# TFMV/quiver

Measured on AMD Instinct MI355X. Metric: flat_cosine_qps_recall_1.0, higher is better.
Workload: dtype f64; 1 GPU; flat cosine scan 10000000x768 fp32, k=10, single query per step, recall 1.0 (exact, bit-identical to the CPU oracle); rows_total=10000000, rows_per_gpu=10000000, dim=768, k=10, scan_streams=1, device=AMD Radeon Graphics (gfx950:sramecc+:xnack-), cus=256, rccl_ranks_seen=0

## Files before the change

### include/qv.h

```cpp
#ifndef QV_H
#define QV_H

#include <stdint.h>
#include <stddef.h>

#ifdef __cplusplus
extern "C" {
#endif

#define QV_ABI_VERSION 4

typedef struct qv_index qv_index;

typedef enum qv_metric {
    QV_COSINE      = 0,
    QV_L2          = 1,
    QV_L2SQ        = 2,
    QV_DOT         = 3,
    QV_L1          = 4,
    QV_COSINE_F32  = 5,
    QV_L2_F32      = 6,
    QV_DOT_F32     = 7,
    QV_L2SQ_F64    = 8,
    QV_METRIC_COUNT = 9
// ... 154 lines not shown
                                       uint32_t candidate_tiles);
int qv_scan_bound8_applies_mq(int metric, uint32_t dim, uint32_t rows, uint32_t nq, uint32_t k, int mode, int plane_mode_mq, int has_plane8);
int qv_scan_bound8_applies_filtered(int metric, uint32_t dim, uint32_t rows, uint32_t nq, uint32_t k, int mode, int plane_mode_filtered, int has_plane8,
                                    uint32_t candidate_tiles);
int qv_scan_bound8_applies(int metric, uint32_t dim, uint32_t rows, uint32_t nq, uint32_t k, int mode, int plane_mode, int has_plane8);
int qv_scan_bound_interval8(int metric, uint32_t dim, int64_t isum, double sq, double qn, double qres, double rn, float rscale8, float rres8, float* d_lo, float* d_hi);
int qv_scan_quantize_row8(uint32_t dim, const float* row, int8_t* out_bytes, float* out_scale, float* out_res);
int qv_scan_bound_applies(int metric, uint32_t dim, uint32_t rows, uint32_t nq, uint32_t k, int mode, int has_plane);
int qv_scan_bound_applies_filtered(int metric, uint32_t dim, uint32_t rows, uint32_t nq, uint32_t k, int mode, int has_plane, uint32_t candidate_tiles);
int qv_scan_route(int metric, uint32_t dim, uint32_t rows, uint32_t nq, uint32_t k, int cus, int tickets, int bound_mode, int plane_mode, int has_plane, int has_plane8,
                  uint32_t candidate_tiles);
int qv_scan_route_ex(int metric, uint32_t dim, uint32_t rows, uint32_t nq, uint32_t k, int cus, int tickets, int bound_mode, int plane_mode, int has_plane, int has_plane8,
                     uint32_t candidate_tiles, int plane_mode_filtered);
int qv_scan_bound_interval(int metric, uint32_t dim, float s, double qn, double rn, float rres, float* d_lo, float* d_hi);
int qv_scan_bound_interval_l2(uint32_t dim, float s, double qn, double rn, float rres, float* d_lo, float* d_hi);
#define QV_DEBUG_RNORM 0
#define QV_DEBUG_RRES  1
#define QV_DEBUG_PLANE 2
#define QV_DEBUG_ROWMAJ16 3
int qv_index_debug_read(qv_index* idx, int what, void* out, size_t bytes);

int qv_index_search_batched_device(qv_index* idx, const float* d_queries, uint32_t nq, uint32_t k,
                                   uint32_t* d_rows_out, float* d_dist_out, uint32_t* d_redo_flags_out, void* stream);

int qv_distance_rows(qv_index* idx, const float* query, const uint32_t* rows, uint32_t n, float* dist_out);
int qv_distance_rows_device(qv_index* idx, const float* d_query, const uint32_t* d_rows, uint32_t n,
                            float* d_dist_out, void* stream);

int qv_distance_pairs(qv_metric metric, const float* a, const float* b, uint32_t n, uint32_t dim,
                      float* dist_out, int device);
// ... 94 lines not shown
```

### quiver_amd/_lib.py

```python
from __future__ import annotations

import ctypes as C
import os

_HERE = os.path.dirname(os.path.abspath(__file__))
LIB_PATH = os.environ.get("QV_LIB_PATH") or os.path.join(_HERE, "lib", "libqv.so")

QV_OK = 0
QV_ERR_INVALID_ARG, QV_ERR_DIM_MISMATCH, QV_ERR_K_NOT_POSITIVE, QV_ERR_OUT_OF_RANGE = -1, -2, -3, -4
QV_ERR_NO_DEVICE, QV_ERR_DEVICE, QV_ERR_OOM, QV_ERR_UNSUPPORTED = -5, -6, -7, -8
QV_FLAG_ROWMAJOR = 1
QV_FLAG_BF16_ROWS = 2
QV_FLAG_NO_SCAN_PLANE = 4
QV_FLAG_L2_SCAN_PLANE = 8
QV_FLAG_GRAPH_PLANE = 16
QV_GRAPH_REJECT_AUTO, QV_GRAPH_REJECT_ALWAYS, QV_GRAPH_REJECT_NEVER = 0, 1, 2
QV_DEBUG_RNORM, QV_DEBUG_RRES, QV_DEBUG_PLANE, QV_DEBUG_ROWMAJ16 = 0, 1, 2, 3
QV_RULE_L2_PLANES = 0x101
QV_BOUND_SCAN_AUTO, QV_BOUND_SCAN_ALWAYS, QV_BOUND_SCAN_NEVER = 0, 1, 2
QV_FILTERED_BATCH_AUTO, QV_FILTERED_BATCH_ALWAYS, QV_FILTERED_BATCH_NEVER = 0, 1, 2
QV_COL_F64, QV_COL_U32 = 0, 1
QV_SET_AND, QV_SET_OR, QV_SET_ANDNOT = 0, 1, 2
QV_SHARDED_PEER_COPY = 1 << 32

# ... 65 lines not shown
    "qv_merge_topk_device": (C.c_int, [C.c_void_p, C.c_void_p, C.c_uint32, C.c_uint32, C.c_void_p, C.c_void_p, C.c_void_p]),
    "qv_merge_topk_shards_device": (C.c_int, [C.c_void_p, C.c_void_p, C.c_uint32, C.c_uint32, C.c_uint32, C.c_void_p, C.c_void_p, C.c_void_p]),
    "qv_index_set_filter": (C.c_int, [C.c_void_p, C.c_int]),
    "qv_index_set_filtered_batch": (C.c_int, [C.c_void_p, C.c_int, C.c_uint32]),
    "qv_index_filtered_batch_stats": (C.c_int, [C.c_void_p, C.POINTER(C.c_uint64)]),
    "qv_batched_applies_filtered": (C.c_int, [C.c_int, C.c_uint32, C.c_uint64, C.c_uint32, C.c_uint32, C.c_int, C.c_int, C.c_uint32]),
    "qv_batched_filter_route": (C.c_int, [C.c_int, C.c_uint32, C.c_uint64, C.c_uint32, C.c_uint32, C.c_int, C.c_int, C.c_int, _u32p, C.POINTER(C.c_int)]),
    "qv_batched_sample_plan": (C.c_int, [C.c_void_p, C.c_uint32, C.c_uint32, _u32p, _u32p, _u32p]),
    "qv_sharded_set_filter": (C.c_int, [C.c_void_p, C.c_int]),
    "qv_index_set_bound_scan": (C.c_int, [C.c_void_p, C.c_int]),
    "qv_sharded_set_bound_scan": (C.c_int, [C.c_void_p, C.c_int]),
    "qv_index_bound_scan_stats": (C.c_int, [C.c_void_p, C.POINTER(C.c_uint64)]),
    "qv_sharded_bound_scan_stats": (C.c_int, [C.c_void_p, C.POINTER(C.c_uint64)]),
    "qv_scan_bound_interval": (C.c_int, [C.c_int, C.c_uint32, C.c_float, C.c_double, C.c_double, C.c_float, _f32p, _f32p]),
    "qv_scan_bound_interval_l2": (C.c_int, [C.c_uint32, C.c_float, C.c_double, C.c_double, C.c_float, _f32p, _f32p]),
    "qv_index_set_bound_plane": (C.c_int, [C.c_void_p, C.c_int]),
    "qv_sharded_set_bound_plane": (C.c_int, [C.c_void_p, C.c_int]),
    "qv_index_bound_scan8_stats": (C.c_int, [C.c_void_p, C.POINTER(C.c_uint64)]),
    "qv_sharded_bound_scan8_stats": (C.c_int, [C.c_void_p, C.POINTER(C.c_uint64)]),
    "qv_index_set_bound_plane_filtered": (C.c_int, [C.c_void_p, C.c_int]),
    "qv_index_set_bound_plane_mq": (C.c_int, [C.c_void_p, C.c_int]),
    "qv_sharded_set_bound_plane_mq": (C.c_int, [C.c_void_p, C.c_int]),
    "qv_index_set_bound_plane_filtered_mq": (C.c_int, [C.c_void_p, C.c_int]),
    "qv_scan_bound8_applies_filtered_mq": (C.c_int, [C.c_int, C.c_uint32, C.c_uint32, C.c_uint32, C.c_uint32, C.c_int, C.c_int, C.c_int, C.c_uint32]),
    "qv_scan_bound8_applies_mq": (C.c_int, [C.c_int, C.c_uint32, C.c_uint32, C.c_uint32, C.c_uint32, C.c_int, C.c_int, C.c_int]),
    "qv_scan_bound8_applies_filtered": (C.c_int, [C.c_int, C.c_uint32, C.c_uint32, C.c_uint32, C.c_uint32, C.c_int, C.c_int, C.c_int, C.c_uint32]),
    "qv_scan_route_ex": (C.c_int, [C.c_int, C.c_uint32, C.c_uint32, C.c_uint32, C.c_uint32, C.c_int, C.c_int, C.c_int, C.c_int, C.c_int, C.c_int, C.c_uint32, C.c_int]),
    "qv_scan_bound8_applies": (C.c_int, [C.c_int, C.c_uint32, C.c_uint32, C.c_uint32, C.c_uint32, C.c_int, C.c_int, C.c_int]),
    "qv_scan_bound_interval8": (C.c_int, [C.c_int, C.c_uint32, C.c_int64, C.c_double, C.c_double, C.c_double, C.c_double, C.c_float, C.c_float, _f32p, _f32p]),
    "qv_scan_quantize_row8": (C.c_int, [C.c_uint32, C.c_void_p, C.c_void_p, _f32p, _f32p]),
# ... 88 lines not shown
```

### quiver_amd/csrc/qv_api.cpp

```cpp
#include "qv_api_internal.h"

#include <atomic>

namespace {
thread_local char g_err[512] = "";

}

int qv_fail(int code, const char* fmt, ...) {
    va_list ap; va_start(ap, fmt);
    vsnprintf(g_err, sizeof(g_err), fmt, ap);
    va_end(ap);
    return code;
}

namespace {

int acquire_ctx(qv_index* idx, SearchCtx** out) {
    {
        std::lock_guard<std::mutex> g(idx->ctx_mu);
        if (!idx->free_ctx.empty()) { *out = idx->free_ctx.back(); idx->free_ctx.pop_back(); return QV_OK; }
    }
    SearchCtx* c = new (std::nothrow) SearchCtx();
    if (!c) return fail(QV_ERR_OOM, "out of host memory");
// ... 1687 lines not shown
    return qv::host_quantize_row8(dim, row, out_bytes, out_scale, out_res);
}

int qv_scan_bound_interval(int metric, uint32_t dim, float s, double qn, double rn, float rres, float* d_lo, float* d_hi) {
    if (metric != QV_COSINE && metric != QV_DOT)
        return fail(QV_ERR_UNSUPPORTED, "the bound scan's metrics are cosine, dot and l2, and this function serves cosine and dot (l2: qv_scan_bound_interval_l2); got %d", metric);
    if (!d_lo || !d_hi || dim == 0) return fail(QV_ERR_INVALID_ARG, "d_lo/d_hi is null or dim is 0");
    return qv::host_bound_interval(metric, dim, s, qn, rn, rres, d_lo, d_hi);
}

int qv_scan_bound_interval_l2(uint32_t dim, float s, double qn, double rn, float rres, float* d_lo, float* d_hi) {
    if (!d_lo || !d_hi || dim == 0) return fail(QV_ERR_INVALID_ARG, "d_lo/d_hi is null or dim is 0");
    return qv::host_bound_interval(QV_L2, dim, s, qn, rn, rres, d_lo, d_hi);
}

int qv_index_debug_read(qv_index* idx, int what, void* out, size_t bytes) {
    if (!idx) return fail(QV_ERR_INVALID_ARG, "index is null");
    const int m = idx->metric;
    const bool f64norm = m == QV_COSINE || m == QV_DOT || m == QV_L2 || m == QV_L2SQ;
    const size_t tiles = ((size_t)idx->n_rows + 63) / 64;
    const void* src = nullptr; size_t need = 0;
    if (what == QV_DEBUG_RNORM) {
        if (!f64norm && m != QV_COSINE_F32) return fail(QV_ERR_UNSUPPORTED, "metric %d keeps no row norms", m);
        src = idx->d_rnorm; need = tiles * 64 * sizeof(double);
    } else if (what == QV_DEBUG_RRES) {
        if (!f64norm) return fail(QV_ERR_UNSUPPORTED, "metric %d keeps no bfloat16 residuals", m);
        src = idx->d_rres; need = tiles * 64 * sizeof(float);
    } else if (what == QV_DEBUG_PLANE) {
        if (!idx->wants_plane() || (tiles && !idx->d_bf16)) return fail(QV_ERR_UNSUPPORTED, "this index keeps no bfloat16 copy");
        src = idx->d_bf16; need = tiles * idx->bf16_tile_bytes();
// ... 183 lines not shown
```

### quiver_amd/csrc/qv_bound.h

```cpp
#pragma once
#include "qv_kernels.h"
#include "qv_filter.h"

namespace qv {

__host__ __device__ static inline double bound_scan_gamma(uint32_t dim) { return filter_gamma(dim, 0) * (1.0 + 1e-6) + 5e-7 + 1e-12; }

__host__ __device__ static inline bool bound_scan_norm_ok(double n, uint32_t dim) { return n >= (double)filter_tiny_norm(dim) && n < 1.0e18; }

constexpr double kBoundL2Theta = 1.2e-7, kBoundL2NormSlack = 2e-12;
__host__ __device__ __forceinline__ bool bound_l2_ends(double s, double m, double qn, double rn, float& d_lo, float& d_hi) {
    const double A = __builtin_fma(qn, qn, rn * rn);
    const double c = A - 2.0 * s, w = 2.0 * m + kBoundL2NormSlack * A;
    const double e_lo = c - w, e_hi = c + w;
    if (!(e_hi >= 0.0)) { d_lo = -__builtin_inff(); d_hi = __builtin_nanf(""); return false; }
    QConst qc; qc.qn = qn; qc.qn32 = 0.0f;
    d_lo = finalize<QV_L2>((e_lo > 0.0 ? e_lo : 0.0) * ((1.0 - kBoundL2Theta) * (1.0 - 1e-9)), qc, rn);
    d_hi = finalize<QV_L2>(e_hi * ((1.0 + kBoundL2Theta) * (1.0 + 1e-9)), qc, rn);
    return true;
}

template <int M>
__host__ __device__ __forceinline__ bool bound_scan_interval(float s, double qn, double rn, float rres, uint32_t dim, double gamma, float& d_lo, float& d_hi) {
    static_assert(M == QV_COSINE || M == QV_DOT || M == QV_L2, "the bound scan's metrics");
// ... 38 lines not shown
                                                              float& d_lo, float& d_hi) {
    static_assert(M == QV_COSINE || M == QV_DOT || M == QV_L2, "the bound scan's metrics");
    const double rr = (double)rres8, sc = (double)rscale;
    const bool sure = bound_scan_norm_ok(rn, dim) && bound_scan_norm_ok(qn, dim) && rr >= 0.0 && rr < 1.0e18 && qres >= 0.0 && qres < 1.0e18 &&
                      sq > 0.0 && sq < 1.0e36 && sc > 0.0 && sc < 1.0e36;
    if (!sure) { d_lo = -__builtin_inff(); d_hi = __builtin_nanf(""); return false; }
    const double s = sq * sc * (double)isum;
    const double m = (qn * rr + qres * (rn + rr) + 1e-12 * (qn + qres) * (rn + rr)) * (1.0 + 1e-9);
    if constexpr (M == QV_L2) return bound_l2_ends(s, m, qn, rn, d_lo, d_hi);
    QConst qc; qc.qn = qn; qc.qn32 = 0.0f;
    d_lo = finalize<M>(s + m, qc, rn);
    d_hi = finalize<M>(s - m, qc, rn);
    return true;
}

}
```

### quiver_amd/csrc/qv_bound_scan.hip

```cpp
#include "qv_kernels.h"
#include "qv_bound.h"

namespace qv {

typedef uint32_t u4 __attribute__((ext_vector_type(4)));
constexpr uint32_t kBoundCandCap = 4096;
constexpr uint32_t kBoundMaxDim = 4096;
struct BoundCtrl { uint32_t thr_inv, cand_cnt, ticket, flag; };

template <int U, bool QN>
__device__ __forceinline__ void bound_block(const u4* __restrict__ p, const float* __restrict__ q_lds, uint32_t s0, float& acc, double& qa) {
    u4 x[2 * U];
#pragma unroll
    for (int u = 0; u < U; u++) {
        x[2 * u] = __builtin_nontemporal_load(&p[(size_t)(s0 + u) * 128]);
        x[2 * u + 1] = __builtin_nontemporal_load(&p[(size_t)(s0 + u) * 128 + 32]);
    }
    __builtin_amdgcn_sched_barrier(0);
#pragma unroll
    for (int u = 0; u < U; u++) {
        const f4* qq = reinterpret_cast<const f4*>(q_lds + (size_t)(s0 + u) * 16);
#pragma unroll
        for (int h = 0; h < 2; h++) {
            const u4 w = x[2 * u + h];
// ... 123 lines not shown
        const uint32_t xs[4] = {x.x, x.y, x.z, x.w};
#pragma unroll
        for (int j = 0; j < 4; j++) {
            const bool c = xs[j] <= H && xs[j] != 0xFFFFFFFFu;
            const uint64_t m = __ballot(c);
            if (m) {
                uint32_t b0 = 0;
                if (lane == (uint32_t)__builtin_ctzll(m)) b0 = atomicAdd(cnt, (uint32_t)__builtin_popcountll(m));
                b0 = __builtin_amdgcn_readlane(b0, (uint32_t)__builtin_ctzll(m));
                const uint32_t slot = b0 + (uint32_t)__builtin_popcountll(m & ((1ull << lane) - 1ull));
                if (c && slot < kBoundCandCap) cand[slot] = i + (uint32_t)j;
            }
        }
    }
}
__global__ void __launch_bounds__(256)
k_bound_collect(const uint32_t* __restrict__ lo_all, uint32_t n , BoundCtrl* __restrict__ ctrl, uint32_t* __restrict__ cand,
                const uint32_t* __restrict__ gate = nullptr ) {
    if (gate != nullptr && *gate == 0u) return;
    const uint32_t inv = ctrl->thr_inv;
    if (inv == 0u) return;
    bound_collect(lo_all, n, ~inv, &ctrl->cand_cnt, cand);
}

template <int M, typename F>
__device__ __forceinline__ void bound_rescore_query(const IndexView& v, const float* __restrict__ query, uint32_t k, uint32_t cnt, bool has_H, const uint32_t* __restrict__ cand,
                                                    uint32_t* __restrict__ rows_out, float* __restrict__ dist_out, F decided) {
    using Q = typename MT<M>::Q;
    extern __shared__ __align__(16) unsigned char smem[];
    Q* q_lds = reinterpret_cast<Q*>(smem);
    uint64_t* wl = reinterpret_cast<uint64_t*>(smem + (((size_t)v.dim4 * 4 * sizeof(Q)) + 15) / 16 * 16);
    __shared__ double s_qn;
    const uint32_t lane = lane_id();
    const uint32_t wave = __builtin_amdgcn_readfirstlane(threadIdx.x >> 6);
    const uint32_t ns = cnt < kBoundCandCap ? cnt : kBoundCandCap, kth = k - 1;
    stage_query<M>(q_lds, query, v.dim, v.dim4);
    __syncthreads();
    const f4* tiles = reinterpret_cast<const f4*>(v.tiles);
// ... 24 lines not shown
        else list_insert(list, thr, key, kth, lane);
    }
    __syncthreads();
    wl[wave * 64 + lane] = list;
    __syncthreads();
    if (wave == 0) {
        for (uint32_t w = 1; w < kScanWaves; w++) list_insert(list, thr, lane < k ? wl[w * 64 + lane] : kDeadKey, kth, lane);
        if (lane < k) {
            const bool dead = list == kDeadKey;
            rows_out[lane] = dead ? 0xFFFFFFFFu : (uint32_t)list;
            dist_out[lane] = dead ? __uint_as_float(0x7F800000u) : unord_f32((uint32_t)(list >> 32));
        }
    }
}

constexpr uint32_t kBoundRescoreGrid = 64;
template <int M, bool P8 = false>
__global__ void __launch_bounds__(kScanBlock)
k_bound_rescore(IndexView v, const float* __restrict__ query, uint32_t k, BoundCtrl* __restrict__ ctrl, const uint32_t* __restrict__ cand,
                uint32_t* __restrict__ stats, uint32_t* __restrict__ rows_out, float* __restrict__ dist_out, uint32_t* gate, BoundCtrl* next,
                uint64_t* __restrict__ partial ) {
    if (gate != nullptr && *gate == 0u) return;
    using Q = typename MT<M>::Q;
    extern __shared__ __align__(16) unsigned char smem[];
    Q* q_lds = reinterpret_cast<Q*>(smem);
    const size_t q_bytes = (((size_t)v.dim4 * 4 * sizeof(Q)) + 15) / 16 * 16;
    uint64_t* wl = reinterpret_cast<uint64_t*>(smem + q_bytes);
    float* rbuf = reinterpret_cast<float*>(smem + q_bytes + (size_t)kScanWaves * 64 * sizeof(uint64_t));
    __shared__ double s_qn;
    __shared__ uint32_t s_last;
    const uint32_t cnt = ctrl->cand_cnt, thr_inv = ctrl->thr_inv;
    const uint32_t lane = lane_id();
    const uint32_t wave = __builtin_amdgcn_readfirstlane(threadIdx.x >> 6);
    const uint32_t ns = cnt < kBoundCandCap ? cnt : kBoundCandCap, kth = k - 1;
    const uint32_t active = std::max(1u, std::min((uint32_t)gridDim.x, (ns + kScanWaves - 1) / kScanWaves));
    const bool idle = blockIdx.x >= active;
    if (idle) {
        if (threadIdx.x == 0) s_last = atomicAdd(&ctrl->ticket, 1u) == gridDim.x - 1 ? 1u : 0u;
        __syncthreads();
        if (!s_last) return;
    }
    stage_query<M>(q_lds, query, v.dim, v.dim4);
    __syncthreads();
    if (wave == kScanWaves - 1) {
        double ma = 0.0;
        for (uint32_t i = 0; i < v.dim; i++) { const double a = (double)q_lds[i]; ma = __builtin_fma(a, a, ma); }
        if (lane == 0) s_qn = __builtin_sqrt(ma);
    }
    __syncthreads();
    const double qn = s_qn;
    const bool hand_back = cnt > kBoundCandCap || thr_inv == 0u || !bound_scan_norm_ok(qn, v.dim);
    uint64_t list = kDeadKey, thr = kDeadKey;
    if (!hand_back && !idle) {
        QConst qc; qc.qn = 0.0; qc.qn32 = 0.0f;
        if constexpr (M == QV_COSINE) qc.qn = qn;
        const f4* tiles = reinterpret_cast<const f4*>(v.tiles);
        f4* mine = reinterpret_cast<f4*>(rbuf + (size_t)wave * v.dim4 * 4);
        bool first = true;
        for (uint32_t i = blockIdx.x * kScanWaves + wave; i < ns; i += active * kScanWaves) {
            const uint32_t row = cand[i];
            const f4* src = tiles + (size_t)(row >> 6) * v.dim4 * 64 + (row & 63);
            double rn = 0.0;
            if constexpr (MT<M>::needs_rnorm) rn = v.rnorm[row];
            for (uint32_t c0 = 0; c0 < v.dim4; c0 += 256) {
                f4 x[4];
#pragma unroll
                for (uint32_t u = 0; u < 4; u++) { const uint32_t c = c0 + u * 64 + lane; if (c < v.dim4) x[u] = __builtin_nontemporal_load(&src[(size_t)c * 64]); }
#pragma unroll
                for (uint32_t u = 0; u < 4; u++) { const uint32_t c = c0 + u * 64 + lane; if (c < v.dim4) mine[c] = x[u]; }
            }
            __builtin_amdgcn_fence(__ATOMIC_RELEASE, "wavefront");
            __builtin_amdgcn_wave_barrier();
            __builtin_amdgcn_fence(__ATOMIC_ACQUIRE, "wavefront");
            typename MT<M>::A acc = 0;
            for (uint32_t c = 0; c < v.dim4; c++) {
                const f4 r = mine[c];
                const Q* qq = q_lds + (size_t)c * 4;
                acc1<M>(acc, qq[0], r.x); acc1<M>(acc, qq[1], r.y); acc1<M>(acc, qq[2], r.z); acc1<M>(acc, qq[3], r.w);
            }
            __builtin_amdgcn_fence(__ATOMIC_RELEASE, "wavefront");
            __builtin_amdgcn_wave_barrier();
            const uint64_t key = lane == 0 ? make_key(finalize<M>(acc, qc, rn), row) : kDeadKey;
            if (first) { list = wave_sort64(key, lane); thr = readlane64(list, kth); first = false; }
            else list_insert(list, thr, key, kth, lane);
        }
    }
    wl[wave * 64 + lane] = list;
    __syncthreads();
    if (wave == 0 && !idle) {
        if (!hand_back) {
            for (uint32_t w = 1; w < kScanWaves; w++) list_insert(list, thr, lane < k ? wl[w * 64 + lane] : kDeadKey, kth, lane);
            uint64_t* out = partial + (size_t)blockIdx.x * k;
            if (lane < k) (void)atomicExch(reinterpret_cast<unsigned long long*>(&out[lane]), (unsigned long long)list);
            asm volatile("s_waitcnt vmcnt(0)" ::: "memory");
        }
        uint32_t last = 0;
        if (lane == 0) last = atomicAdd(&ctrl->ticket, 1u) == gridDim.x - 1 ? 1u : 0u;
        last = __builtin_amdgcn_readfirstlane(last);
        if (lane == 0) s_last = last;
    }
    __syncthreads();
    if (!s_last) return;
    if (threadIdx.x == 0) {
        ctrl->ticket = 0;
        if constexpr (P8) {
            stats[kBound8StatsWord] = cnt;
            if (hand_back) (void)atomicAdd(&stats[kBound8StatsWord + 1], 1u);
            (void)atomicAdd(&stats[kBound8StatsWord + 2], 1u);
            if (!hand_back) { stats[0] = cnt; (void)atomicAdd(&stats[2], 1u); next->flag = 0u; }
        } else {
            stats[0] = cnt;
            if (hand_back) (void)atomicAdd(&stats[1], 1u);
            (void)atomicAdd(&stats[2], 1u);
            if (gate != nullptr) *gate = 0u;
        }
        ctrl->flag = hand_back ? 1u : 0u;
        ctrl->cand_cnt = 0; ctrl->thr_inv = 0;
    }
    if (hand_back) return;
    merge_lists_last_workgroup(partial, active, k, rows_out, dist_out);
}

typedef int i32;
template <int U>
__device__ __forceinline__ void bound8_block(const u4* __restrict__ p, const u4* __restrict__ qh, const u4* __restrict__ ql, uint32_t s0, i32 (&acc)[4]) {
    u4 x[U];
#pragma unroll
    for (int u = 0; u < U; u++) x[u] = __builtin_nontemporal_load(&p[(size_t)(s0 + u) * 64]);
    __builtin_amdgcn_sched_barrier(0);
#pragma unroll
    for (int u = 0; u < U; u++) {
        const u4 h = qh[s0 + u], l = ql[s0 + u];
        acc[0] = __builtin_amdgcn_sdot4((i32)h.x, (i32)x[u].x, acc[0], false);
        acc[1] = __builtin_amdgcn_sdot4((i32)h.y, (i32)x[u].y, acc[1], false);
        acc[0] = __builtin_amdgcn_sdot4((i32)h.z, (i32)x[u].z, acc[0], false);
// ... 535 lines not shown
    const BoundFilterFloor& g = kBoundFilterFloor[rules][cls];
    const uint64_t n_tiles = ((uint64_t)a.n_rows + 63) / 64, ct = std::min<uint64_t>(a.candidate_tiles, n_tiles);
    if (ct == 0 || a.dim < g.min_dim || g.min_rows == 0 || a.n_rows < g.min_rows) return false;
    const bool big = g.big_rows != 0 && a.n_rows >= g.big_rows;
    return ct * 10 >= n_tiles * (big ? g.big_tenths : g.tenths) && (big || g.small_k == 0 || a.k <= g.small_k);
}
BoundStages bound_scan_decide(const BoundAsk& a, const BoundKnobs& knobs) {
    const int scan = bound_scan_mode(knobs.scan);
    if (scan == 2 || !bound_scan_kernels_serve(a)) return BoundStages::none;
    if (scan != 1 && !bound_auto(a, a.rule_metric == QV_RULE_L2_PLANES ? kRulesBf16L2 : kRulesBf16)) return BoundStages::none;
    const int plane = bound_plane_mode(bound_form(a), knobs.plane[bound_form(a)]);
    if (plane == 2 || !a.has_plane8) return BoundStages::bf16;
    return plane == 1 || bound_auto(a, kRulesPlane8) ? BoundStages::plane8_first : BoundStages::bf16;
}
size_t bound_scan_workspace_bytes(const ScanPlan& p, uint32_t k, uint32_t n_tiles) {
    return ((size_t)p.grid * k * sizeof(uint64_t) + 255) / 256 * 256 + 512 + (size_t)kBoundCandCap * sizeof(uint32_t) + (size_t)n_tiles * 64 * sizeof(uint32_t);
}
hipError_t launch_bound_scan(const IndexView& v, const ScanPlan& p, const float* d_query, uint32_t k, void* d_ws, uint32_t* d_ctrl, uint32_t* d_stats,
                             uint32_t* d_rows_out, float* d_dist_out, const uint32_t** gate_out, hipStream_t s, bool masked, bool plane8_first) {
    if (!bound_scan_kernels_serve(bound_ask(v, 1, k, kBoundNoFilter)) || !d_ctrl || !d_stats) return hipErrorInvalidValue;
    if (plane8_first && !v.plane8) return hipErrorInvalidValue;
    const uint32_t grid = p.grid;
    char* w = static_cast<char*>(d_ws);
    uint64_t* partial = reinterpret_cast<uint64_t*>(w); w += ((size_t)p.grid * k * sizeof(uint64_t) + 255) / 256 * 256;
    uint32_t* seed_rows = reinterpret_cast<uint32_t*>(w); w += 256;
    float* seed_dist = reinterpret_cast<float*>(w); w += 256;
    uint32_t* cand = reinterpret_cast<uint32_t*>(w); w += (size_t)kBoundCandCap * sizeof(uint32_t);
    uint32_t* lo_all = reinterpret_cast<uint32_t*>(w);
    const uint32_t n_pad = v.n_tiles * 64, cgrid = std::min(1024u, (n_pad + 1023u) / 1024u);
    BoundCtrl* ctrl = reinterpret_cast<BoundCtrl*>(d_ctrl);
    const size_t lds1 = (size_t)v.dim * sizeof(float) + (size_t)kScanWaves * 64 * sizeof(uint64_t);
    const size_t lds2 = query_lds_bytes(v.metric, v.dim4) + (size_t)kScanWaves * 64 * sizeof(uint64_t) + (size_t)kScanWaves * v.dim4 * 4 * sizeof(float);
    const uint32_t rgrid = std::min(kBoundRescoreGrid, grid);
    const size_t lds8 = (size_t)v.dim * 2 + (size_t)kScanWaves * 64 * sizeof(uint64_t);
    auto run = [&](auto Mc, auto Mk) -> hipError_t {
        constexpr int M = decltype(Mc)::value;
        constexpr bool MASKED = decltype(Mk)::value;
        auto attrs = [&](auto scan, size_t lds_scan, auto rescore) -> hipError_t {
            const hipError_t e = set_lds(scan, lds_scan);
            return e != hipSuccess ? e : set_lds(rescore, lds2);
        };
        auto stage = [&](auto scan, size_t lds_scan, auto rescore, BoundCtrl* c, uint32_t* gate, BoundCtrl* next, auto... scan_gate) {
            hipLaunchKernelGGL(scan, dim3(grid), dim3(kScanBlock), lds_scan, s, v, d_query, k, c, lo_all, partial, seed_rows, seed_dist, scan_gate...);
            hipLaunchKernelGGL(k_bound_collect, dim3(cgrid), dim3(256), 0, s, lo_all, n_pad, c, cand, (const uint32_t*)gate);
            hipLaunchKernelGGL(rescore, dim3(rgrid), dim3(kScanBlock), lds2, s, v, d_query, k, c, cand, d_stats, d_rows_out, d_dist_out, gate, next, partial);
        };
        const uint32_t* const no_gate = nullptr;
        hipError_t e = attrs(k_bound_scan<M, MASKED>, lds1, k_bound_rescore<M>);
        if (e == hipSuccess && plane8_first) e = attrs(k_bound_scan8<M, MASKED>, lds8, k_bound_rescore<M, true>);
        if (e != hipSuccess) return e;
        if (plane8_first) {
            BoundCtrl* ctrl8 = ctrl + 1;
            uint32_t* gate8 = &ctrl8->flag;
            stage(k_bound_scan8<M, MASKED>, lds8, k_bound_rescore<M, true>, ctrl8, (uint32_t*)nullptr, ctrl);
            stage(k_bound_scan<M, MASKED>, lds1, k_bound_rescore<M>, ctrl, gate8, (BoundCtrl*)nullptr, (const uint32_t*)gate8);
        } else stage(k_bound_scan<M, MASKED>, lds1, k_bound_rescore<M>, ctrl, (uint32_t*)nullptr, (BoundCtrl*)nullptr, no_gate);
        return hipSuccess;
    };
    auto run_metric = [&](auto Mk) -> hipError_t {
        return v.metric == QV_COSINE ? run(std::integral_constant<int, QV_COSINE>{}, Mk)
// ... 6 lines not shown
}
int host_bound_interval(int metric, uint32_t dim, float s, double qn, double rn, float rres, float* d_lo, float* d_hi) {
    const double gamma = bound_scan_gamma(dim);
    const bool sure = metric == QV_COSINE ? bound_scan_interval<QV_COSINE>(s, qn, rn, rres, dim, gamma, *d_lo, *d_hi)
                    : metric == QV_DOT  ? bound_scan_interval<QV_DOT>(s, qn, rn, rres, dim, gamma, *d_lo, *d_hi)
                                        : bound_scan_interval<QV_L2>(s, qn, rn, rres, dim, gamma, *d_lo, *d_hi);
    return sure ? 0 : 1;
}

int host_bound_interval8(int metric, uint32_t dim, long long isum, double sq, double qn, double qres, double rn, float rscale, float rres8, float* d_lo, float* d_hi) {
    const bool sure = metric == QV_COSINE ? bound_scan_interval8<QV_COSINE>(isum, sq, qn, qres, rn, rscale, rres8, dim, *d_lo, *d_hi)
                    : metric == QV_DOT  ? bound_scan_interval8<QV_DOT>(isum, sq, qn, qres, rn, rscale, rres8, dim, *d_lo, *d_hi)
                                        : bound_scan_interval8<QV_L2>(isum, sq, qn, qres, rn, rscale, rres8, dim, *d_lo, *d_hi);
    return sure ? 0 : 1;
}
int host_quantize_row8(uint32_t dim, const float* row, int8_t* out_bytes, float* out_scale, float* out_res) {
    float maxabs = 0.f; bool bad = false; double n2 = 0.0;
    for (uint32_t i = 0; i < dim; i++) {
        bad |= !((row[i] - row[i]) == 0.0f);
        maxabs = __builtin_fmaxf(maxabs, __builtin_fabsf(row[i]));
        n2 = __builtin_fma((double)row[i], (double)row[i], n2);
    }
    const float scale = bad ? 0.0f : bound8_scale(maxabs);
    double s2 = 0.0;
    for (uint32_t i = 0; i < dim; i++) {
        const int b = scale > 0.0f ? bound8_quant(row[i], scale) : 0;
        const double d = (double)row[i] - (double)scale * (double)b;
        s2 = __builtin_fma(d, d, s2);
        out_bytes[i] = (int8_t)b;
    }
// ... 79 lines not shown
```

### quiver_amd/csrc/qv_device.h

```cpp
#pragma once
#include <hip/hip_runtime.h>
#include <stdint.h>

namespace qv {

constexpr int kTileRows = 64;
constexpr int kMaxFusedK = 64;
constexpr int kMaxWideK = 128;
constexpr int kMaxBatchedK = 4096;
constexpr int kMaxSelectK = 8192;
constexpr uint64_t kDeadKey = ~0ull;

struct IndexView {
    float*    tiles;
    double*   rnorm;
    uint64_t* alive;
    float*    rres;
    float*    rowmaj;
    uint16_t* bf16;
    uint32_t  dim;
    uint32_t  dim4;
    uint32_t  n_rows;
    uint32_t  n_tiles;
    int       metric;
// ... 130 lines not shown
BoundKnobs bound_knobs(const IndexView& v);
int bound_scan_mode(int mode);
size_t bound_scan_workspace_bytes(const ScanPlan& p, uint32_t k, uint32_t n_tiles);
hipError_t launch_bound_scan(const IndexView& v, const ScanPlan& p, const float* d_query, uint32_t k, void* d_ws, uint32_t* d_ctrl, uint32_t* d_stats,
                             uint32_t* d_rows_out, float* d_dist_out, const uint32_t** gate_out, hipStream_t s,
                             bool masked = false,
                             bool plane8_first = false);
size_t bound_scan_mq_workspace_bytes(const ScanPlan& p, uint32_t nq, uint32_t k, uint32_t n_tiles, uint32_t dim);
hipError_t launch_bound_scan_mq(const IndexView& v, const ScanPlan& p, const float* d_queries, uint32_t nq, uint32_t k, void* d_ws, uint32_t* d_ctrl, uint32_t* d_stats,
                                uint32_t* d_rows_out, float* d_dist_out, hipStream_t s,
                                const RowSetRef* h_sets = nullptr,
                                bool plane8_first = false);
int host_bound_interval(int metric, uint32_t dim, float s, double qn, double rn, float rres, float* d_lo, float* d_hi);
int host_bound_interval8(int metric, uint32_t dim, long long isum, double sq, double qn, double qres, double rn, float rscale, float rres8, float* d_lo, float* d_hi);
int host_quantize_row8(uint32_t dim, const float* row, int8_t* out_bytes, float* out_scale, float* out_res);
constexpr uint32_t kBound8StatsWord = 4;
constexpr uint32_t kBoundCtrlWord = 16;
bool flat_split_applies(const IndexView& v, uint32_t nq, uint32_t k);
size_t redo_workspace_bytes(const ScanPlan& p, uint32_t nq, uint32_t k);
hipError_t launch_flat_redo_flagged(const IndexView& v, const ScanPlan& p, const float* d_queries, uint32_t nq, uint32_t k, uint32_t k_stride, const uint32_t* d_flags,
                                    void* d_ws, uint32_t* d_rows_out, float* d_dist_out, hipStream_t s,
                                    const RowSetRef* h_sets = nullptr);
bool flat_small_applies(const IndexView& v, uint32_t nq, uint32_t k);
size_t flat_small_workspace_bytes(uint32_t nq, uint32_t k);
hipError_t launch_flat_small(const IndexView& v, const float* d_queries, uint32_t nq, uint32_t k, void* d_ws, uint32_t* d_tickets, uint32_t* d_rows_out, float* d_dist_out,
                             uint32_t* done_flag, uint32_t done_seq, hipStream_t s, hipEvent_t ev0 = nullptr, hipEvent_t ev1 = nullptr);
hipError_t launch_merge_shards(const uint32_t* d_packed, const uint32_t* d_bases, uint32_t n_lists, uint32_t nq, uint32_t k,
                               uint32_t* d_rows_out, float* d_dist_out, hipStream_t s, uint32_t planes = 0 );
size_t merge_ranked_workspace_bytes(uint64_t n_keys);
hipError_t launch_merge_ranked(const uint32_t* d_packed, const uint32_t* d_bases, uint32_t n_lists, uint32_t nq, uint32_t q, uint32_t kcap, uint32_t planes,
// ... 132 lines not shown
```

Baseline: 797.1 queries/s.

## Fuse bound-scan candidate collection into a batched multi-row rescore kernel

Drops the separate collect kernel: the rescore kernel now reads the per-tile lower-bound words itself in tile batches, queues surviving rows in LDS, and drains them by staging several rows per wave into padded LDS before scoring them with a software-pipelined dot loop. The query norm is computed during the first rescore pass rather than in a separate serial step. The final merge is done by the last workgroup, tracked through a split ticket word. The aim is to cut one kernel launch and a global candidate round-trip and to rescore with more parallelism, at the cost of much larger LDS use (up to 159 KiB), a wider rescore grid and more complex control flow.

```diff
diff --git a/include/qv.h b/include/qv.h
--- a/include/qv.h
+++ b/include/qv.h
@@ -192,6 +192,9 @@
                      uint32_t candidate_tiles, int plane_mode_filtered);
 int qv_scan_bound_interval(int metric, uint32_t dim, float s, double qn, double rn, float rres, float* d_lo, float* d_hi);
 int qv_scan_bound_interval_l2(uint32_t dim, float s, double qn, double rn, float rres, float* d_lo, float* d_hi);
+int qv_scan_bound_finish_shape(uint32_t* batch_tiles, uint32_t* max_grid);
+int qv_scan_bound_finish_batches(uint32_t wg, uint32_t grid, uint32_t n_tiles, uint32_t* batches);
+int qv_scan_bound_finish_tiles(uint32_t wg, uint32_t grid, uint32_t batch, uint32_t n_tiles, uint32_t* tiles, uint32_t n_slots);
 #define QV_DEBUG_RNORM 0
 #define QV_DEBUG_RRES  1
 #define QV_DEBUG_PLANE 2
diff --git a/quiver_amd/_lib.py b/quiver_amd/_lib.py
--- a/quiver_amd/_lib.py
+++ b/quiver_amd/_lib.py
@@ -103,6 +103,9 @@
     "qv_sharded_bound_scan_stats": (C.c_int, [C.c_void_p, C.POINTER(C.c_uint64)]),
     "qv_scan_bound_interval": (C.c_int, [C.c_int, C.c_uint32, C.c_float, C.c_double, C.c_double, C.c_float, _f32p, _f32p]),
     "qv_scan_bound_interval_l2": (C.c_int, [C.c_uint32, C.c_float, C.c_double, C.c_double, C.c_float, _f32p, _f32p]),
+    "qv_scan_bound_finish_shape": (C.c_int, [_u32p, _u32p]),
+    "qv_scan_bound_finish_batches": (C.c_int, [C.c_uint32, C.c_uint32, C.c_uint32, _u32p]),
+    "qv_scan_bound_finish_tiles": (C.c_int, [C.c_uint32, C.c_uint32, C.c_uint32, C.c_uint32, _u32p, C.c_uint32]),
     "qv_index_set_bound_plane": (C.c_int, [C.c_void_p, C.c_int]),
     "qv_sharded_set_bound_plane": (C.c_int, [C.c_void_p, C.c_int]),
     "qv_index_bound_scan8_stats": (C.c_int, [C.c_void_p, C.POINTER(C.c_uint64)]),
diff --git a/quiver_amd/csrc/qv_api.cpp b/quiver_amd/csrc/qv_api.cpp
--- a/quiver_amd/csrc/qv_api.cpp
+++ b/quiver_amd/csrc/qv_api.cpp
@@ -1725,6 +1725,25 @@
     return qv::host_bound_interval(QV_L2, dim, s, qn, rn, rres, d_lo, d_hi);
 }
 
+int qv_scan_bound_finish_shape(uint32_t* batch_tiles, uint32_t* max_grid) {
+    if (!batch_tiles || !max_grid) return fail(QV_ERR_INVALID_ARG, "batch_tiles/max_grid is null");
+    *batch_tiles = qv::host_bound_finish_batch_tiles(); *max_grid = qv::host_bound_finish_max_grid();
+    return QV_OK;
+}
+
+int qv_scan_bound_finish_batches(uint32_t wg, uint32_t grid, uint32_t n_tiles, uint32_t* batches) {
+    if (!batches || grid == 0 || wg >= grid) return fail(QV_ERR_INVALID_ARG, "batches is null, grid is 0 or wg is not below grid");
+    *batches = qv::host_bound_finish_batches(wg, grid, n_tiles);
+    return QV_OK;
+}
+
+int qv_scan_bound_finish_tiles(uint32_t wg, uint32_t grid, uint32_t batch, uint32_t n_tiles, uint32_t* tiles, uint32_t n_slots) {
+    if (!tiles || grid == 0 || wg >= grid) return fail(QV_ERR_INVALID_ARG, "tiles is null, grid is 0 or wg is not below grid");
+    if (n_slots > qv::host_bound_finish_batch_tiles()) return fail(QV_ERR_INVALID_ARG, "a batch has %u slots; %u asked for", qv::host_bound_finish_batch_tiles(), n_slots);
+    for (uint32_t i = 0; i < n_slots; i++) tiles[i] = qv::host_bound_finish_tile(wg, grid, batch, i, n_tiles);
+    return QV_OK;
+}
+
 int qv_index_debug_read(qv_index* idx, int what, void* out, size_t bytes) {
     if (!idx) return fail(QV_ERR_INVALID_ARG, "index is null");
     const int m = idx->metric;
diff --git a/quiver_amd/csrc/qv_bound.h b/quiver_amd/csrc/qv_bound.h
--- a/quiver_amd/csrc/qv_bound.h
+++ b/quiver_amd/csrc/qv_bound.h
@@ -76,4 +76,14 @@
     return true;
 }
 
+constexpr uint32_t kBoundFinishBatchTiles = 128;
+__host__ __device__ static inline uint32_t bound_finish_batches(uint32_t b, uint32_t G, uint32_t n_tiles) {
+    const uint64_t own = b < n_tiles ? ((uint64_t)(n_tiles - b) + G - 1) / G : 0ull;
+    return (uint32_t)((own + kBoundFinishBatchTiles - 1) / kBoundFinishBatchTiles);
 }
+__host__ __device__ static inline uint32_t bound_finish_tile(uint32_t b, uint32_t G, uint32_t batch, uint32_t i, uint32_t n_tiles) {
+    const uint64_t t = ((uint64_t)batch * kBoundFinishBatchTiles + i) * G + b;
+    return t < n_tiles ? (uint32_t)t : n_tiles;
+}
+
+}
diff --git a/quiver_amd/csrc/qv_bound_scan.hip b/quiver_amd/csrc/qv_bound_scan.hip
--- a/quiver_amd/csrc/qv_bound_scan.hip
+++ b/quiver_amd/csrc/qv_bound_scan.hip
@@ -161,14 +161,6 @@
         }
     }
 }
-__global__ void __launch_bounds__(256)
-k_bound_collect(const uint32_t* __restrict__ lo_all, uint32_t n , BoundCtrl* __restrict__ ctrl, uint32_t* __restrict__ cand,
-                const uint32_t* __restrict__ gate = nullptr ) {
-    if (gate != nullptr && *gate == 0u) return;
-    const uint32_t inv = ctrl->thr_inv;
-    if (inv == 0u) return;
-    bound_collect(lo_all, n, ~inv, &ctrl->cand_cnt, cand);
-}
 
 template <int M, typename F>
 __device__ __forceinline__ void bound_rescore_query(const IndexView& v, const float* __restrict__ query, uint32_t k, uint32_t cnt, bool has_H, const uint32_t* __restrict__ cand,
@@ -223,94 +215,201 @@
     }
 }
 
-constexpr uint32_t kBoundRescoreGrid = 64;
+constexpr uint32_t kBoundFinishGrid = 256;
+constexpr uint32_t kBoundFinishMaxRows = 8;
+constexpr uint32_t kBoundFinishBatchWords = kBoundFinishBatchTiles * 64;
+constexpr uint32_t kBoundFinishDrainAt = 2048;
+constexpr uint32_t kBoundFinishQueue = kBoundFinishDrainAt + kBoundFinishBatchWords;
+constexpr uint32_t kBoundFinishMergeCap = kBoundFinishQueue * sizeof(uint32_t) / sizeof(uint64_t);
+constexpr size_t kBoundFinishLds = 159 * 1024;
+static_assert(kBoundFinishGrid < 65536u, "the ticket word's halves");
+static_assert(kBoundFinishMergeCap >= kBoundCandCap, "a search that is answered re-scored at most kBoundCandCap rows: their keys fit the merge");
+__host__ __device__ static inline uint32_t bound_finish_stride(uint32_t dim4) { return dim4 | 1u; }
+static inline size_t bound_finish_fixed_lds(int metric, uint32_t dim4) {
+    return query_lds_bytes(metric, dim4) + (size_t)kScanWaves * 64 * sizeof(uint64_t) + (size_t)kBoundFinishQueue * sizeof(uint32_t);
+}
 template <int M, bool P8 = false>
 __global__ void __launch_bounds__(kScanBlock)
-k_bound_rescore(IndexView v, const float* __restrict__ query, uint32_t k, BoundCtrl* __restrict__ ctrl, const uint32_t* __restrict__ cand,
-                uint32_t* __restrict__ stats, uint32_t* __restrict__ rows_out, float* __restrict__ dist_out, uint32_t* gate, BoundCtrl* next,
-                uint64_t* __restrict__ partial ) {
+k_bound_rescore(IndexView v, const float* __restrict__ query, uint32_t k, BoundCtrl* ctrl, const uint32_t* __restrict__ lo_all , uint32_t R,
+                double* qn_ws , uint32_t* __restrict__ stats, uint32_t* __restrict__ rows_out, float* __restrict__ dist_out, uint32_t* gate, BoundCtrl* next,
+                uint64_t* partial ) {
     if (gate != nullptr && *gate == 0u) return;
     using Q = typename MT<M>::Q;
+    using A = typename MT<M>::A;
     extern __shared__ __align__(16) unsigned char smem[];
     Q* q_lds = reinterpret_cast<Q*>(smem);
     const size_t q_bytes = (((size_t)v.dim4 * 4 * sizeof(Q)) + 15) / 16 * 16;
     uint64_t* wl = reinterpret_cast<uint64_t*>(smem + q_bytes);
-    float* rbuf = reinterpret_cast<float*>(smem + q_bytes + (size_t)kScanWaves * 64 * sizeof(uint64_t));
-    __shared__ double s_qn;
-    __shared__ uint32_t s_last;
-    const uint32_t cnt = ctrl->cand_cnt, thr_inv = ctrl->thr_inv;
+    uint32_t* queue = reinterpret_cast<uint32_t*>(smem + q_bytes + (size_t)kScanWaves * 64 * sizeof(uint64_t));
+    uint64_t* surv = reinterpret_cast<uint64_t*>(queue);
+    f4* rbuf = reinterpret_cast<f4*>(queue + kBoundFinishQueue);
+    __shared__ uint32_t s_cnt, s_over, s_last, s_lists, s_hand, s_live;
+    const uint32_t thr_inv = ctrl->thr_inv;
     const uint32_t lane = lane_id();
     const uint32_t wave = __builtin_amdgcn_readfirstlane(threadIdx.x >> 6);
-    const uint32_t ns = cnt < kBoundCandCap ? cnt : kBoundCandCap, kth = k - 1;
-    const uint32_t active = std::max(1u, std::min((uint32_t)gridDim.x, (ns + kScanWaves - 1) / kScanWaves));
-    const bool idle = blockIdx.x >= active;
-    if (idle) {
-        if (threadIdx.x == 0) s_last = atomicAdd(&ctrl->ticket, 1u) == gridDim.x - 1 ? 1u : 0u;
+    const uint32_t kth = k - 1, G = gridDim.x, b = blockIdx.x, nt = v.n_tiles, dim4 = v.dim4;
+    const uint32_t stride = bound_finish_stride(dim4);
+    f4* mine = rbuf + (size_t)wave * R * stride;
+    const f4* tiles = reinterpret_cast<const f4*>(v.tiles);
+    uint64_t list = kDeadKey, thr = kDeadKey;
+    bool first = true, staged = false, have_qn = false, over = false;
+    double qn = 0.0;
+    if (threadIdx.x == 0) { s_cnt = 0; s_over = 0; }
+    __syncthreads();
+
+    auto drain = [&](uint32_t m) {
+        if (threadIdx.x == 0) {
+            s_cnt = 0;
+            if (atomicAdd(&ctrl->cand_cnt, m) + m > kBoundCandCap) s_over = 1;
+        }
         __syncthreads();
-        if (!s_last) return;
-    }
-    stage_query<M>(q_lds, query, v.dim, v.dim4);
-    __syncthreads();
-    if (wave == kScanWaves - 1) {
-        double ma = 0.0;
-        for (uint32_t i = 0; i < v.dim; i++) { const double a = (double)q_lds[i]; ma = __builtin_fma(a, a, ma); }
-        if (lane == 0) s_qn = __builtin_sqrt(ma);
-    }
-    __syncthreads();
-    const double qn = s_qn;
-    const bool hand_back = cnt > kBoundCandCap || thr_inv == 0u || !bound_scan_norm_ok(qn, v.dim);
-    uint64_t list = kDeadKey, thr = kDeadKey;
-    if (!hand_back && !idle) {
-        QConst qc; qc.qn = 0.0; qc.qn32 = 0.0f;
-        if constexpr (M == QV_COSINE) qc.qn = qn;
-        const f4* tiles = reinterpret_cast<const f4*>(v.tiles);
-        f4* mine = reinterpret_cast<f4*>(rbuf + (size_t)wave * v.dim4 * 4);
-        bool first = true;
-        for (uint32_t i = blockIdx.x * kScanWaves + wave; i < ns; i += active * kScanWaves) {
-            const uint32_t row = cand[i];
-            const f4* src = tiles + (size_t)(row >> 6) * v.dim4 * 64 + (row & 63);
-            double rn = 0.0;
-            if constexpr (MT<M>::needs_rnorm) rn = v.rnorm[row];
-            for (uint32_t c0 = 0; c0 < v.dim4; c0 += 256) {
-                f4 x[4];
-#pragma unroll
-                for (uint32_t u = 0; u < 4; u++) { const uint32_t c = c0 + u * 64 + lane; if (c < v.dim4) x[u] = __builtin_nontemporal_load(&src[(size_t)c * 64]); }
-#pragma unroll
-                for (uint32_t u = 0; u < 4; u++) { const uint32_t c = c0 + u * 64 + lane; if (c < v.dim4) mine[c] = x[u]; }
+        over = over || s_over != 0;
+        if (!over) {
+            staged = true;
+            for (uint32_t base = 0; base < m; base += kScanWaves * R) {
+                const uint32_t mr = std::min(m - base, (uint32_t)kScanWaves * R), per = (mr + kScanWaves - 1) / kScanWaves;
+                const uint32_t j0 = wave * per;
+                if (j0 >= mr) continue;
+                const uint32_t nr = std::min(per, mr - j0);
+                auto row_of = [&](uint32_t j) -> uint32_t {
+                    const uint32_t e = queue[base + j0 + j], li = e >> 6;
+                    return bound_finish_tile(b, G, li / kBoundFinishBatchTiles, li % kBoundFinishBatchTiles, nt) * 64u + (e & 63u);
+                };
+                const bool act = lane < nr;
+                const uint32_t row = row_of(act ? lane : 0u);
+                double rn = 0.0;
+                if constexpr (MT<M>::needs_rnorm) rn = v.rnorm[row];
+                const uint32_t total = nr * dim4;
+                for (uint32_t i0 = 0; i0 < total; i0 += 512) {
+                    f4 y[8]; uint32_t dst[8];
+#pragma unroll
+                    for (uint32_t u = 0; u < 8; u++) {
+                        const uint32_t i = i0 + u * 64 + lane;
+                        dst[u] = 0xFFFFFFFFu;
+                        if (i < total) {
+                            const uint32_t j = i / dim4, c = i - j * dim4, rj = row_of(j);
+                            dst[u] = j * stride + c;
+                            y[u] = __builtin_nontemporal_load(&tiles[(size_t)(rj >> 6) * dim4 * 64 + (rj & 63) + (size_t)c * 64]);
+                        }
+                    }
+#pragma unroll
+                    for (uint32_t u = 0; u < 8; u++) if (dst[u] != 0xFFFFFFFFu) mine[dst[u]] = y[u];
+                }
+                __builtin_amdgcn_fence(__ATOMIC_RELEASE, "wavefront");
+                __builtin_amdgcn_wave_barrier();
+                __builtin_amdgcn_fence(__ATOMIC_ACQUIRE, "wavefront");
+                const f4* src = mine + (size_t)(act ? lane : 0u) * stride;
+                auto chain = [&](auto QNc, double& qa) -> A {
+                    constexpr bool QN = decltype(QNc)::value;
+                    A acc = 0;
+                    f4 r[4], r2[4]; Q qv[16], qv2[16];
+                    auto fetch = [&](uint32_t c, f4 (&rr)[4], Q (&qq)[16]) {
+#pragma unroll
+                        for (int u = 0; u < 4; u++) rr[u] = src[c + u];
+#pragma unroll
+                        for (int e = 0; e < 16; e++) qq[e] = q_lds[(size_t)c * 4 + e];
+                    };
+                    auto one = [&](Q a, float x) { acc1<M>(acc, a, x); if constexpr (QN) { const double d = (double)a; qa = __builtin_fma(d, d, qa); } };
+                    auto block = [&](const f4 (&rr)[4], const Q (&qq)[16]) {
+#pragma unroll
+                        for (int u = 0; u < 4; u++) { one(qq[4 * u], rr[u].x); one(qq[4 * u + 1], rr[u].y); one(qq[4 * u + 2], rr[u].z); one(qq[4 * u + 3], rr[u].w); }
+                    };
+                    const uint32_t nblk = dim4 / 4;
+                    uint32_t blk = 0;
+                    if (nblk) fetch(0, r, qv);
+                    for (; blk + 2 <= nblk; blk += 2) {
+                        fetch((blk + 1) * 4, r2, qv2);
+                        __builtin_amdgcn_sched_barrier(0);
+                        block(r, qv);
+                        if (blk + 2 < nblk) fetch((blk + 2) * 4, r, qv);
+                        __builtin_amdgcn_sched_barrier(0);
+                        block(r2, qv2);
+                    }
+                    if (blk < nblk) block(r, qv);
+                    for (uint32_t c = nblk * 4; c < dim4; c++) {
+                        const f4 x = src[c];
+                        const Q* qq = q_lds + (size_t)c * 4;
+                        one(qq[0], x.x); one(qq[1], x.y); one(qq[2], x.z); one(qq[3], x.w);
+                    }
+                    return acc;
+                };
+                A acc;
+                if (!have_qn) { double qa = 0.0; acc = chain(std::true_type{}, qa); qn = __builtin_sqrt(qa); have_qn = true; }
+                else { double none = 0.0; acc = chain(std::false_type{}, none); }
+                __builtin_amdgcn_fence(__ATOMIC_RELEASE, "wavefront");
+                __builtin_amdgcn_wave_barrier();
+                QConst qc; qc.qn = 0.0; qc.qn32 = 0.0f;
+                if constexpr (M == QV_COSINE) qc.qn = qn;
+                const uint64_t key = act ? make_key(finalize<M>(acc, qc, rn), row) : kDeadKey;
+                if (first) { list = wave_sort64(key, lane); thr = readlane64(list, kth); first = false; }
+                else list_insert(list, thr, key, kth, lane);
             }
-            __builtin_amdgcn_fence(__ATOMIC_RELEASE, "wavefront");
-            __builtin_amdgcn_wave_barrier();
-            __builtin_amdgcn_fence(__ATOMIC_ACQUIRE, "wavefront");
-            typename MT<M>::A acc = 0;
-            for (uint32_t c = 0; c < v.dim4; c++) {
-                const f4 r = mine[c];
-                const Q* qq = q_lds + (size_t)c * 4;
-                acc1<M>(acc, qq[0], r.x); acc1<M>(acc, qq[1], r.y); acc1<M>(acc, qq[2], r.z); acc1<M>(acc, qq[3], r.w);
+        }
+        __syncthreads();
+    };
+
+    if (thr_inv != 0u) {
+        const uint32_t H = ~thr_inv;
+        const uint32_t nb = bound_finish_batches(b, G, nt);
+        const uint32_t ti = threadIdx.x >> 4, tw4 = (threadIdx.x & 15u) * 4u;
+        auto request = [&](uint32_t batch, u4 (&x)[8]) {
+#pragma unroll
+            for (uint32_t u = 0; u < 8; u++) {
+                const uint32_t t = batch < nb ? bound_finish_tile(b, G, batch, u * 16 + ti, nt) : nt;
+                x[u] = u4{0xFFFFFFFFu, 0xFFFFFFFFu, 0xFFFFFFFFu, 0xFFFFFFFFu};
+                if (t < nt) x[u] = __builtin_nontemporal_load(reinterpret_cast<const u4*>(lo_all + (size_t)t * 64 + tw4));
             }
-            __builtin_amdgcn_fence(__ATOMIC_RELEASE, "wavefront");
-            __builtin_amdgcn_wave_barrier();
-            const uint64_t key = lane == 0 ? make_key(finalize<M>(acc, qc, rn), row) : kDeadKey;
-            if (first) { list = wave_sort64(key, lane); thr = readlane64(list, kth); first = false; }
-            else list_insert(list, thr, key, kth, lane);
-        }
-    }
-    wl[wave * 64 + lane] = list;
-    __syncthreads();
-    if (wave == 0 && !idle) {
-        if (!hand_back) {
-            for (uint32_t w = 1; w < kScanWaves; w++) list_insert(list, thr, lane < k ? wl[w * 64 + lane] : kDeadKey, kth, lane);
-            uint64_t* out = partial + (size_t)blockIdx.x * k;
-            if (lane < k) (void)atomicExch(reinterpret_cast<unsigned long long*>(&out[lane]), (unsigned long long)list);
-            asm volatile("s_waitcnt vmcnt(0)" ::: "memory");
-        }
-        uint32_t last = 0;
-        if (lane == 0) last = atomicAdd(&ctrl->ticket, 1u) == gridDim.x - 1 ? 1u : 0u;
-        last = __builtin_amdgcn_readfirstlane(last);
-        if (lane == 0) s_last = last;
+        };
+        u4 x[8], xn[8];
+        request(0, x);
+        stage_query<M>(q_lds, query, v.dim, dim4);
+        for (uint32_t batch = 0; batch < nb; batch++) {
+            request(batch + 1, xn);
+            __builtin_amdgcn_sched_barrier(0);
+#pragma unroll
+            for (uint32_t u = 0; u < 8; u++) {
+                const uint32_t xs[4] = {x[u].x, x[u].y, x[u].z, x[u].w};
+#pragma unroll
+                for (uint32_t j = 0; j < 4; j++)
+                    if (xs[j] <= H && xs[j] != 0xFFFFFFFFu) queue[atomicAdd(&s_cnt, 1u)] = ((batch * kBoundFinishBatchTiles + u * 16 + ti) << 6) + tw4 + j;
+            }
+#pragma unroll
+            for (uint32_t u = 0; u < 8; u++) x[u] = xn[u];
+            __syncthreads();
+            const uint32_t fill = s_cnt;
+            __syncthreads();
+            if (fill != 0u && (fill > kBoundFinishDrainAt || batch + 1 == nb)) drain(fill);
+        }
+    }
+
+    if (staged) wl[wave * 64 + lane] = list;
+    __syncthreads();
+    if (wave == 0) {
+        if (staged) for (uint32_t w = 1; w < kScanWaves; w++) list_insert(list, thr, lane < k ? wl[w * 64 + lane] : kDeadKey, kth, lane);
+        uint64_t* out = partial + (size_t)b * k;
+        if (lane < k) (void)atomicExch(reinterpret_cast<unsigned long long*>(&out[lane]), (unsigned long long)list);
+        if (staged && lane == 0) (void)atomicExch(reinterpret_cast<unsigned long long*>(qn_ws), (unsigned long long)__double_as_longlong(qn));
+        asm volatile("s_waitcnt vmcnt(0)" ::: "memory");
+        if (lane == 0) {
+            const uint32_t old = atomicAdd(&ctrl->ticket, staged ? 0x10001u : 1u);
+            s_last = (old & 0xFFFFu) == G - 1 ? 1u : 0u;
+            s_lists = (old >> 16) + (staged ? 1u : 0u);
+        }
     }
     __syncthreads();
     if (!s_last) return;
+    const uint32_t n_lists = s_lists;
+    auto ld = [](const uint64_t* p) -> uint64_t { return __hip_atomic_load(p, __ATOMIC_RELAXED, __HIP_MEMORY_SCOPE_AGENT); };
+    const uint32_t total = G * k;
+    uint64_t key[8];
+#pragma unroll
+    for (uint32_t u = 0; u < 8; u++) { const uint32_t i = u * kScanBlock + threadIdx.x; key[u] = i < total ? ld(partial + i) : kDeadKey; }
     if (threadIdx.x == 0) {
+        const uint32_t cnt = __hip_atomic_load(&ctrl->cand_cnt, __ATOMIC_RELAXED, __HIP_MEMORY_SCOPE_AGENT);
+        const double pq = __longlong_as_double((long long)__hip_atomic_load(reinterpret_cast<unsigned long long*>(qn_ws), __ATOMIC_RELAXED, __HIP_MEMORY_SCOPE_AGENT));
+        const bool hand_back = cnt > kBoundCandCap || thr_inv == 0u || n_lists == 0u || !bound_scan_norm_ok(pq, v.dim);
+        s_hand = hand_back ? 1u : 0u;
+        s_live = 0;
         ctrl->ticket = 0;
         if constexpr (P8) {
             stats[kBound8StatsWord] = cnt;
@@ -326,8 +425,28 @@
         ctrl->flag = hand_back ? 1u : 0u;
         ctrl->cand_cnt = 0; ctrl->thr_inv = 0;
     }
-    if (hand_back) return;
-    merge_lists_last_workgroup(partial, active, k, rows_out, dist_out);
+    __syncthreads();
+    if (s_hand) return;
+    for (uint32_t base = 0; base < total; base += kScanBlock * 8) {
+        if (base != 0) {
+#pragma unroll
+            for (uint32_t u = 0; u < 8; u++) { const uint32_t i = base + u * kScanBlock + threadIdx.x; key[u] = i < total ? ld(partial + i) : kDeadKey; }
+        }
+#pragma unroll
+        for (uint32_t u = 0; u < 8; u++)
+            if (key[u] != kDeadKey) { const uint32_t pos = atomicAdd(&s_live, 1u); if (pos < kBoundFinishMergeCap) surv[pos] = key[u]; }
+    }
+    __syncthreads();
+    if (wave != 0) return;
+    const uint32_t ns = std::min(s_live, kBoundFinishMergeCap);
+    list = wave_sort64(lane < ns ? surv[lane] : kDeadKey, lane);
+    thr = readlane64(list, kth);
+    for (uint32_t base = 64; base < ns; base += 64) list_insert(list, thr, base + lane < ns ? surv[base + lane] : kDeadKey, kth, lane);
+    if (lane < k) {
+        const bool dead = list == kDeadKey;
+        rows_out[lane] = dead ? 0xFFFFFFFFu : (uint32_t)list;
+        dist_out[lane] = dead ? __uint_as_float(0x7F800000u) : unord_f32((uint32_t)(list >> 32));
+    }
 }
 
 typedef int i32;
@@ -893,7 +1012,7 @@
     return plane == 1 || bound_auto(a, kRulesPlane8) ? BoundStages::plane8_first : BoundStages::bf16;
 }
 size_t bound_scan_workspace_bytes(const ScanPlan& p, uint32_t k, uint32_t n_tiles) {
-    return ((size_t)p.grid * k * sizeof(uint64_t) + 255) / 256 * 256 + 512 + (size_t)kBoundCandCap * sizeof(uint32_t) + (size_t)n_tiles * 64 * sizeof(uint32_t);
+    return ((size_t)p.grid * k * sizeof(uint64_t) + 255) / 256 * 256 + 768 + (size_t)n_tiles * 64 * sizeof(uint32_t);
 }
 hipError_t launch_bound_scan(const IndexView& v, const ScanPlan& p, const float* d_query, uint32_t k, void* d_ws, uint32_t* d_ctrl, uint32_t* d_stats,
                              uint32_t* d_rows_out, float* d_dist_out, const uint32_t** gate_out, hipStream_t s, bool masked, bool plane8_first) {
@@ -904,13 +1023,15 @@
     uint64_t* partial = reinterpret_cast<uint64_t*>(w); w += ((size_t)p.grid * k * sizeof(uint64_t) + 255) / 256 * 256;
     uint32_t* seed_rows = reinterpret_cast<uint32_t*>(w); w += 256;
     float* seed_dist = reinterpret_cast<float*>(w); w += 256;
-    uint32_t* cand = reinterpret_cast<uint32_t*>(w); w += (size_t)kBoundCandCap * sizeof(uint32_t);
+    double* qn_ws = reinterpret_cast<double*>(w); w += 256;
     uint32_t* lo_all = reinterpret_cast<uint32_t*>(w);
-    const uint32_t n_pad = v.n_tiles * 64, cgrid = std::min(1024u, (n_pad + 1023u) / 1024u);
     BoundCtrl* ctrl = reinterpret_cast<BoundCtrl*>(d_ctrl);
     const size_t lds1 = (size_t)v.dim * sizeof(float) + (size_t)kScanWaves * 64 * sizeof(uint64_t);
-    const size_t lds2 = query_lds_bytes(v.metric, v.dim4) + (size_t)kScanWaves * 64 * sizeof(uint64_t) + (size_t)kScanWaves * v.dim4 * 4 * sizeof(float);
-    const uint32_t rgrid = std::min(kBoundRescoreGrid, grid);
+    static const uint32_t max_rows = (uint32_t)dev_env_int("QV_BOUND_FINISH_ROWS", (int)kBoundFinishMaxRows), max_grid = (uint32_t)dev_env_int("QV_BOUND_FINISH_GRID", (int)kBoundFinishGrid);
+    const size_t fixed2 = bound_finish_fixed_lds(v.metric, v.dim4), row2 = (size_t)kScanWaves * bound_finish_stride(v.dim4) * sizeof(f4);
+    const uint32_t rrows = (uint32_t)std::max<size_t>(1, std::min<size_t>(std::min(max_rows, kBoundFinishMaxRows), fixed2 < kBoundFinishLds ? (kBoundFinishLds - fixed2) / row2 : 0));
+    const size_t lds2 = fixed2 + rrows * row2;
+    const uint32_t rgrid = std::min(std::min(max_grid, kBoundFinishGrid), grid);
     const size_t lds8 = (size_t)v.dim * 2 + (size_t)kScanWaves * 64 * sizeof(uint64_t);
     auto run = [&](auto Mc, auto Mk) -> hipError_t {
         constexpr int M = decltype(Mc)::value;
@@ -921,8 +1042,7 @@
         };
         auto stage = [&](auto scan, size_t lds_scan, auto rescore, BoundCtrl* c, uint32_t* gate, BoundCtrl* next, auto... scan_gate) {
             hipLaunchKernelGGL(scan, dim3(grid), dim3(kScanBlock), lds_scan, s, v, d_query, k, c, lo_all, partial, seed_rows, seed_dist, scan_gate...);
-            hipLaunchKernelGGL(k_bound_collect, dim3(cgrid), dim3(256), 0, s, lo_all, n_pad, c, cand, (const uint32_t*)gate);
-            hipLaunchKernelGGL(rescore, dim3(rgrid), dim3(kScanBlock), lds2, s, v, d_query, k, c, cand, d_stats, d_rows_out, d_dist_out, gate, next, partial);
+            hipLaunchKernelGGL(rescore, dim3(rgrid), dim3(kScanBlock), lds2, s, v, d_query, k, c, (const uint32_t*)lo_all, rrows, qn_ws, d_stats, d_rows_out, d_dist_out, gate, next, partial);
         };
         const uint32_t* const no_gate = nullptr;
         hipError_t e = attrs(k_bound_scan<M, MASKED>, lds1, k_bound_rescore<M>);
@@ -959,6 +1079,10 @@
                                         : bound_scan_interval8<QV_L2>(isum, sq, qn, qres, rn, rscale, rres8, dim, *d_lo, *d_hi);
     return sure ? 0 : 1;
 }
+uint32_t host_bound_finish_batch_tiles() { return kBoundFinishBatchTiles; }
+uint32_t host_bound_finish_max_grid() { return kBoundFinishGrid; }
+uint32_t host_bound_finish_batches(uint32_t b, uint32_t G, uint32_t n_tiles) { return bound_finish_batches(b, G, n_tiles); }
+uint32_t host_bound_finish_tile(uint32_t b, uint32_t G, uint32_t batch, uint32_t i, uint32_t n_tiles) { return bound_finish_tile(b, G, batch, i, n_tiles); }
 int host_quantize_row8(uint32_t dim, const float* row, int8_t* out_bytes, float* out_scale, float* out_res) {
     float maxabs = 0.f; bool bad = false; double n2 = 0.0;
     for (uint32_t i = 0; i < dim; i++) {
diff --git a/quiver_amd/csrc/qv_device.h b/quiver_amd/csrc/qv_device.h
--- a/quiver_amd/csrc/qv_device.h
+++ b/quiver_amd/csrc/qv_device.h
@@ -168,6 +168,10 @@
 int host_bound_interval(int metric, uint32_t dim, float s, double qn, double rn, float rres, float* d_lo, float* d_hi);
 int host_bound_interval8(int metric, uint32_t dim, long long isum, double sq, double qn, double qres, double rn, float rscale, float rres8, float* d_lo, float* d_hi);
 int host_quantize_row8(uint32_t dim, const float* row, int8_t* out_bytes, float* out_scale, float* out_res);
+uint32_t host_bound_finish_batch_tiles();
+uint32_t host_bound_finish_max_grid();
+uint32_t host_bound_finish_batches(uint32_t b, uint32_t G, uint32_t n_tiles);
+uint32_t host_bound_finish_tile(uint32_t b, uint32_t G, uint32_t batch, uint32_t i, uint32_t n_tiles);
 constexpr uint32_t kBound8StatsWord = 4;
 constexpr uint32_t kBoundCtrlWord = 16;
 bool flat_split_applies(const IndexView& v, uint32_t nq, uint32_t k);
```

After: 800.9 queries/s (median of 6 runs). No clear change (+0.5%).
